# c5shen/WITCH

Measured on AMD Instinct MI355X. Metric: query-seqs aligned/sec (100k queries x 200-HMM eHMM), higher is better.
Workload: dtype f32; 1 GPU; dna_100k_x200; n_queries=100000, n_hmms=200, query_len=150, model_len_min=898, model_len_max=993, k=10, pairs_reported_rank0=20000000, pairs_multidomain_rank0=968, pairs_long_list_rank0=0, pairs_dense_redo_rank0=3, topk_crc32=3263627139

## Files before the change

### include/witch_hip.h

```cpp
#ifndef WITCH_HIP_H
#define WITCH_HIP_H

#include <stdint.h>

#ifdef __cplusplus
extern "C" {
#endif

#define WH_OK          0
#define WH_EINVAL     -1
#define WH_EIO        -2
#define WH_ENODEV     -3
#define WH_EHIP       -4
#define WH_ERANGE     -5
#define WH_ENOMEM     -6

#define WH_ALPH_DNA    0
#define WH_ALPH_RNA    1
#define WH_ALPH_AMINO  2

#define WH_FLAG_REPORTED  1
#define WH_FLAG_MULTI     2
#define WH_FLAG_OVERRIDE  4
#define WH_FLAG_TRUNC     8
// ... 141 lines not shown
int wh_last_score_counters(wh_ehmm *e, int64_t *out8);
int wh_last_region_overflow(wh_ehmm *e, int64_t *out4);
int wh_last_long_query_pairs(wh_ehmm *e, int64_t out[2]);
int wh_last_long_score_pairs(wh_ehmm *e, int64_t out[2]);
int wh_last_long_align_pairs(wh_ehmm *e, int64_t out[2]);

int wh_set_path_buffer(wh_ehmm *e, uint8_t *d_paths);
int wh_set_path_buffer16(wh_ehmm *e, uint16_t *d_paths);

int wh_last_queue_reruns(wh_ehmm *e);

int wh_consensus(wh_ehmm *e, const int64_t *offsets, int64_t nq, const int64_t *qpair_off,
                 const int32_t *pair_h, const double *pair_w, const int64_t *col_offsets, const int32_t *cols,
                 const int64_t *ret_off, const int32_t *retained, const int32_t *nongaps,
                 int32_t backbone_length, int32_t *out, int32_t *minmax);
int wh_consensus_dev(wh_ehmm *e, const int64_t *d_offsets, int64_t nq, int32_t max_len, const int64_t *d_qpair_off,
                     const int32_t *d_pair_h, const double *d_pair_w, const int64_t *d_col_offsets,
                     const int32_t *d_cols, const int64_t *d_ret_off, const int32_t *d_retained,
                     const int32_t *d_nongaps, int32_t backbone_length, int32_t max_pairs_per_query,
                     int32_t *d_out, int32_t *d_minmax, void *stream);

int wh_last_kernel_ms(wh_ehmm *e, int which, double *ms, int *launches);
int wh_last_score_launches(wh_ehmm *e, int32_t *cells_per_lane, int32_t *kind, double *ms, int cap);
int wh_set_timing(wh_ehmm *e, int enabled);
int wh_set_option(wh_ehmm *e, const char *name, const char *value);

int wh_merge(int device, const uint8_t *q_text, const int64_t *q_off, int64_t nq, const int32_t *codes, const int32_t *q_row,
             const uint8_t *backbone, int32_t nb, int32_t B, uint8_t **out_full, uint8_t **out_masked, int64_t *out_rows,
             int64_t *out_width);
int wh_merge_sharded(int device, const uint8_t *q_text, const int64_t *q_off, int64_t nq, const int32_t *codes, const int32_t *q_row,
                     const uint8_t *backbone, int32_t nb, int32_t B, int32_t *widths_local, const int32_t *widths_global,
                     uint8_t **out_full, uint8_t **out_masked, int64_t *out_rows, int64_t *out_width);

#define WH_MSA_TRIM   1
#define WH_MSA_NO_LDS 2
#define WH_MSA_CONS_HMMER 4
int wh_msa(wh_ehmm *e, const uint8_t *residues, const int64_t *offsets, const uint8_t *text, int64_t nq, int32_t h,
           int32_t flags, int64_t *out_W, uint8_t **out_rows, uint8_t **out_pp_rows, uint8_t **out_pp_cons, uint8_t **out_rf,
           int32_t **out_matmap, int64_t *out_pathless);
int wh_msa_dev(wh_ehmm *e, const int32_t *d_cols, const float *d_pp, const uint8_t *d_text, const int64_t *d_offsets,
               int64_t nq, int64_t total_residues, int32_t h, int32_t flags, int64_t *out_W, uint8_t **out_rows,
               uint8_t **out_pp_rows, uint8_t **out_pp_cons, uint8_t **out_rf, int32_t **out_matmap, int64_t *out_pathless,
               void *stream);

int wh_msa_mapali(wh_ehmm *e, const uint8_t *residues, const int64_t *offsets, const uint8_t *text, int64_t nq, int32_t h,
                  int32_t flags, const uint8_t *map_rows, int64_t n_map, int64_t alen, int64_t *out_W, uint8_t **out_rows,
// ... 90 lines not shown
```

### witch_amd/_lib.py

```python
from __future__ import annotations

import ctypes as C
import os
import subprocess

_HERE = os.path.dirname(os.path.abspath(__file__))
LIB_PATH = os.path.join(_HERE, "libwitch_hip.so")
CSRC = os.path.join(_HERE, "csrc")

WH_MAX_ENVELOPES = 16
FLAG_REPORTED, FLAG_MULTI, FLAG_OVERRIDE, FLAG_TRUNC, FLAG_EXACT = 1, 2, 4, 8, 16
FLAG_FILTERED = 32
BIAS_FILTER_ON = 2
STAGE_MSV, STAGE_BIAS, STAGE_VIT, STAGE_VIT_RAN, STAGE_FWD = 1, 2, 4, 8, 16
VIT_NOT_RUN, VIT_OVERFLOW, MSV_OVERFLOW = -32769, 32768, -1
ALPH_DNA, ALPH_RNA, ALPH_AMINO = 0, 1, 2
WH_OK, WH_EINVAL, WH_EIO, WH_ENODEV, WH_EHIP, WH_ERANGE, WH_ENOMEM = 0, -1, -2, -3, -4, -5, -6
WH_BUILD_STATS, WH_BUILD_CALIB_NO_LDS = 1, 4
WH_MSA_TRIM, WH_MSA_NO_LDS, WH_MSA_CONS_HMMER = 1, 2, 4
WH_LENMODEL_ENVELOPE, WH_LENMODEL_SEQUENCE = 0, 1
PATH_P2_WIN, PATH_P2_FULL, PATH_P4_W256, PATH_P4_W512, PATH_P4_WFAIL, PATH_P4_FULL, PATH_DENSE, PATH_MULTI = 1, 2, 4, 8, 16, 32, 64, 128


class WitchHipError(RuntimeError):
# ... 118 lines not shown
    "wh_seq_expect": (C.c_int, [_P, _P, _P, C.c_int64, _P, C.c_int64, _P]),
    "wh_seq_expect_dev": (C.c_int, [_P, _P, _P, C.c_int64, C.c_int64, C.c_int32, _P, C.c_int64, _P, _P]),
    "wh_seq_expect_host": (C.c_int, [C.POINTER(C.c_char_p), C.c_int, _P, _P, C.c_int64, _P, C.c_int64, _P]),
    "wh_seq_table": (C.c_int, [_P, _P, _P, C.c_int64, _P, _P, _P, _P, C.c_int64]),
    "wh_seq_table_dev": (C.c_int, [_P, _P, _P, C.c_int64, C.c_int64, C.c_int32, _P, _P, _P, _P, C.c_int64, _P]),
    "wh_seq_table_host": (C.c_int, [C.c_int, _P, _P, _P, C.c_int64, _P, _P, _P, _P, _P, C.c_int64]),
    "wh_last_seq_table_status": (C.c_int, [_P, _P]),
    "wh_ehmm_evparams": (C.c_int, [_P, _P, _P, _P]),
    "wh_hmm_evparams": (C.c_int, [C.c_char_p, C.POINTER(C.c_float), C.POINTER(C.c_float), C.POINTER(C.c_int32)]),
    "wh_consensus": (C.c_int, [_P, _P, C.c_int64, _P, _P, _P, _P, _P, _P, _P, _P, C.c_int32, _P, _P]),
    "wh_consensus_dev": (C.c_int, [_P, _P, C.c_int64, C.c_int32, _P, _P, _P, _P, _P, _P, _P, _P, C.c_int32, C.c_int32, _P, _P, _P]),
    "wh_last_align_status": (C.c_int, [_P, C.POINTER(C.c_int64), C.POINTER(C.c_int64), _P, C.c_int64]),
    "wh_last_align_paths": (C.c_int, [_P, _P]),
    "wh_last_score_paths": (C.c_int, [_P, _P]),
    "wh_last_score_counters": (C.c_int, [_P, _P]),
    "wh_set_path_buffer": (C.c_int, [_P, _P]),
    "wh_set_path_buffer16": (C.c_int, [_P, _P]),
    "wh_last_queue_reruns": (C.c_int, [_P]),
    "wh_last_region_overflow": (C.c_int, [_P, _P]),
    "wh_last_long_query_pairs": (C.c_int, [_P, _P]),
    "wh_last_long_score_pairs": (C.c_int, [_P, _P]),
    "wh_last_long_align_pairs": (C.c_int, [_P, _P]),
    "wh_last_score_launches": (C.c_int, [_P, _P, _P, _P, C.c_int]),
    "wh_last_kernel_ms": (C.c_int, [_P, C.c_int, C.POINTER(C.c_double), C.POINTER(C.c_int)]),
    "wh_set_timing": (C.c_int, [_P, C.c_int]),
    "wh_set_option": (C.c_int, [_P, C.c_char_p, C.c_char_p]),
}

_LIB = None


def build(force: bool = False, verbose: bool = False) -> str:
    cmd = ["make", "-C", CSRC, "-j4"] + (["-B"] if force else [])
    r = subprocess.run(cmd, stdout=subprocess.PIPE, stderr=subprocess.STDOUT, text=True)
    if verbose or r.returncode != 0:
        print(r.stdout)
    if r.returncode != 0:
        raise WitchHipError("building libwitch_hip.so failed:\n" + r.stdout[-4000:])
    return LIB_PATH


def lib():
    global _LIB
    if _LIB is None:
        if not os.path.exists(LIB_PATH):
            raise WitchHipError(
# ... 20 lines not shown
```

### witch_amd/csrc/wh_api.hip

```cpp
#include <atomic>
#include <chrono>
#include <memory>
#include <thread>

#include "wh_host.h"

static int g_device = -1;

extern "C" {

const char *wh_version(void) { return "witch_hip 0.1.0 (gfx950)"; }
const char *wh_last_error(void) { return wh::last_error(); }

int wh_init(int device) {
  int n = 0;
  if (hipGetDeviceCount(&n) != hipSuccess || n <= 0) {
    set_error("no HIP device visible");
    return WH_ENODEV;
  }
  if (device < 0 || device >= n) {
    set_error("device %d out of range (0..%d)", device, n - 1);
    return WH_EINVAL;
  }
  HIPCHK(hipSetDevice(device));
// ... 278 lines not shown
  out[0] = e->last_long_align[0]; out[1] = e->last_long_align[1];
  return WH_OK;
}

int wh_last_queue_reruns(wh_ehmm *e) {
  if (!e) { set_error("wh_last_queue_reruns: null handle"); return WH_EINVAL; }
  return e->last_queue_reruns;
}

int wh_last_score_launches(wh_ehmm *e, int32_t *cells_per_lane, int32_t *kind, double *ms, int cap) {
  if (!e || cap < 0) { set_error("wh_last_score_launches: bad argument"); return WH_EINVAL; }
  const int n = e->cls_n > 0 ? e->cls_n - 1 : 0;
  for (int t = 0; t < n && t < cap; t++) {
    HIPCHK(hipEventSynchronize(e->cls_ev[(size_t)t + 1]));
    float f = 0.f;
    HIPCHK(hipEventElapsedTime(&f, e->cls_ev[(size_t)t], e->cls_ev[(size_t)t + 1]));
    if (cells_per_lane) cells_per_lane[t] = e->cls_q[(size_t)t];
    if (kind) kind[t] = e->cls_kind[(size_t)t];
    if (ms) ms[t] = f;
  }
  return n;
}

int wh_last_kernel_ms(wh_ehmm *e, int which, double *ms, int *launches) {
  if (!e || which < 0 || which >= wh_ehmm::kTimers) return WH_EINVAL;
  KernelTimer &t = e->timers[which];
  if (t.pending) {
    HIPCHK(hipEventSynchronize(t.e1));
    float f = 0.f;
    HIPCHK(hipEventElapsedTime(&f, t.e0, t.e1));
    t.ms = f;
    t.pending = false;
  }
  if (ms) *ms = t.ms;
  if (launches) *launches = t.launches;
  return WH_OK;
}

int wh_merge(int device, const uint8_t *q_text, const int64_t *q_off, int64_t nq, const int32_t *codes, const int32_t *q_row,
             const uint8_t *backbone, int32_t nb, int32_t B, uint8_t **out_full, uint8_t **out_masked, int64_t *out_rows,
             int64_t *out_width) {
  return wh_merge_sharded(device, q_text, q_off, nq, codes, q_row, backbone, nb, B, nullptr, nullptr, out_full, out_masked, out_rows, out_width);
}

int wh_merge_sharded(int device, const uint8_t *q_text, const int64_t *q_off, int64_t nq, const int32_t *codes, const int32_t *q_row,
                     const uint8_t *backbone, int32_t nb, int32_t B, int32_t *widths_local, const int32_t *widths_global,
// ... 281 lines not shown
```

### witch_amd/csrc/wh_host.h

```cpp
#pragma once
#include <hip/hip_runtime.h>

#include <algorithm>
#include <cmath>
#include <cstdio>
#include <cstdlib>
#include <cstring>
#include <map>
#include <memory>
#include <vector>

#include "wh_devbuf.h"
#include "wh_knobs.h"
#include "wh_launch.h"
#include "wh_plan.h"

namespace wh {
const char *last_error();
}

using namespace wh;

struct KernelTimer {
  hipEvent_t e0 = nullptr, e1 = nullptr;
// ... 89 lines not shown
  uint16_t *path_buf16 = nullptr;
  static const int kStagingSlots = 11;
  DevBuf staging[kStagingSlots];
  DevBuf d_rkeys, d_rorder, d_rchunks, d_qorder, d_order, d_items, d_recs, d_spec, d_back, d_cwj, d_cwv, d_cwn, d_crow;
  uint32_t degen[32];
  struct FilterStateDelete { void operator()(FilterState *f) const; };
  std::unique_ptr<FilterState, FilterStateDelete> filter;
  struct SeqTabStateDelete { void operator()(SeqTabState *f) const; };
  std::unique_ptr<SeqTabState, SeqTabStateDelete> seqtab;
  struct DisplayStateDelete { void operator()(DisplayState *f) const; };
  std::unique_ptr<DisplayState, DisplayStateDelete> display;
  bool timing = false;
  static const int kTimers = 10;
  KernelTimer timers[kTimers];
  int max_M = 0;
  int max_Q = 4;
  int last_align_redo = 0;
  int last_align_unaligned = 0;
  int64_t last_align_paths[4] = {0, 0, 0, 0};
  std::vector<int64_t> last_unaligned_pairs;
  std::vector<hipEvent_t> cls_ev;
  std::vector<int> cls_q, cls_kind;
  int cls_n = 0;
  int *counter(int slot) const { return (int *)d_counter.p + slot; }
  ResolveFeedback *d_feedback() const { return (ResolveFeedback *)counter(kSlotResolveFeedback); }
};

static inline int max_query_len(const int64_t *offsets, int64_t nq) {
  int64_t m = 0;
  for (int64_t i = 0; i < nq; i++) m = std::max(m, offsets[i + 1] - offsets[i]);
  return (int)m;
}
static inline int check_residues(int Kp, const uint8_t *residues, int64_t total) {
  for (int64_t i = 0; i < total; i++)
    if (residues[i] >= Kp) { set_error("residue code %d at position %lld is not in the alphabet", residues[i], (long long)i); return WH_EINVAL; }
  return WH_OK;
}

struct Staging {
  wh_ehmm *e;
  int rc = WH_OK, next = 0, nback = 0;
  struct { void *host; const void *dev; size_t bytes; } back[wh_ehmm::kStagingSlots];
  explicit Staging(wh_ehmm *handle) : e(handle) {}
  template <class T> const T *in(const T *host, size_t bytes, size_t pad = 0) { return (const T *)take((void *)host, bytes, pad, true, false); }
  template <class T> T *out(T *host, size_t bytes, size_t pad = 0) { return (T *)take(host, bytes, pad, false, true); }
  template <class T> T *inout(T *host, size_t bytes, size_t pad = 0) { return (T *)take(host, bytes, pad, true, true); }
// ... 169 lines not shown
```

### witch_amd/csrc/wh_host_score.hip

```cpp
#include "wh_host.h"

static const int kStagedMaxBatches = 1 << 15;
static const int kStagedQB = 48;

static int resolve_main_cap(int max_M) {
  const size_t per_wave = (kLdsBudget - resolve_lds_header_bytes(0)) / (size_t)resolve_waves_per_cu();
  int lo = 1, hi = 1 << 20;
  while (lo < hi) {
    const int mid = lo + (hi - lo + 1) / 2;
    if (resolve_lds_bytes(mid, max_M) <= per_wave) lo = mid; else hi = mid - 1;
  }
  return lo;
}

static ScoreCall score_call(wh_ehmm *e, const uint8_t *d_residues, const int64_t *d_offsets, int64_t nq, int64_t total_residues, int32_t max_len,
                            int32_t *d_decibits, uint8_t *d_flags, float *d_fwd_bits, wh_pair_detail *d_detail, void *stream) {
  ScoreCall c = {e, (hipStream_t)stream, d_residues, d_offsets, nq, total_residues, max_len, d_decibits, d_flags, d_fwd_bits, d_detail};
  c.Lc = std::max(max_len, 1);
  c.H = (int)e->hmms.size();
  c.npairs_all = nq * (int64_t)c.H;
  const bool fits = resolve_lds_bytes(c.Lc, e->max_M) <= kLdsBudget;
  c.Lmain = fits || e->knobs.no_long_query ? c.Lc : resolve_main_cap(e->max_M);
  c.resolve = !e->knobs.no_resolve && (fits || !e->knobs.no_long_query) && c.npairs_all < 0x7FFFFFFF;
  c.mixed = nq > 0 && total_residues > 0 && (double)max_len > 1.25 * (double)total_residues / (double)nq;
  c.wide_dense = getenv("WH_WIDE_DENSE"); c.wide_no_em_lds = getenv("WH_WIDE_NO_EM_LDS"); c.p2win_force = getenv("WH_P2WIN_FORCE");
  c.res_null2_gather = getenv("WH_RES_NULL2_GATHER"); c.res_no_lds_tables = getenv("WH_RES_NO_LDS_TABLES");
  if (const char *wv = getenv("WH_RES_WAVES")) c.res_waves = std::max(1, atoi(wv));
  c.Ls = main_length_cap(e, c.Lc, false, c.resolve, c.p2win_force);
  return c;
}

struct StagedWaves { int wl, one, both, p2, p4; };
enum class ScoreFamily { PhaseCall, PhaseCallB, TwoQuery, FourEnvelope, PassSync, Staged };
static const char *const kFamilyName[] = {"phase-call", "phase-call(B)", "two-queries-per-wave", "phase-call", "pass-synchronous", "staged"};

struct ScoreClassPlan {
  int Q, list_off, n_list;
  ScoreFamily family;
  LdsPlan b;
  int Klds;
  bool specg;
  int p2win;
  bool use_qorder;
  int QB, n_qblocks, n_items;
  size_t scratch_stride, spec_stride;
  int blocks;
  StagedWaves st;
};

static int cap_waves(const Knobs &kn, int w) { return cap_waves(kn.max_waves, w); }
static size_t score_table_bytes(const wh_ehmm *e, int Q) { return score_table_bytes(e->K, Q); }

static const int G_all = 1, G_most = 4, G_few = 8, G_rare = 32;
static int staged_cand_cap(int G, int per_pair) { return std::min(G * kStagedQB * per_pair, 2048); }
static size_t staged_lds(int Q, int wl, int arrays, int waves, int cand) {
  return lds_bytes(kLdsHeader + (size_t)cand * sizeof(int), (size_t)arrays * Q * kWave * sizeof(float), waves, wl);
}
// ... 17 lines not shown
  const size_t table = score_table_bytes(e, Q);
  ScoreClassPlan p = {};
  p.Q = Q; p.list_off = list_off; p.n_list = n_list;
  ScoreLds l;
  if (!plan_score_lds(plan_knobs(e, c.p2win_force), e->K, Q, Lc, true, &l)) { set_error("query length %d with model class Q=%d does not fit in LDS", c.max_len, Q); return WH_ERANGE; }
  p.b = l.b; p.Klds = l.Klds;
  LdsPlan &b = p.b;
  const bool big = l.big, specg = l.specg, pairk = l.pairk, p2win = l.p2win, p2inpl = l.p2inpl;
  bool quadk = false;
  if ((kn.kernel == 10 || kn.kernel == 11) && !e->st_off && !big && !pairk && !specg && !kn.dbg && (Q == 8 || Q == 12 || Q == 16 || Q == 20 || Q == 24) &&
      plan_staged(e, Q, Lc, &p.st)) {
    p.family = ScoreFamily::Staged;
    b.SP = row_stride(Lc); b.wave_lds = p.st.wl;
    p.QB = kStagedQB; p.n_qblocks = (int)((nq + p.QB - 1) / p.QB); p.n_items = n_list * p.n_qblocks;
    p.scratch_stride = (size_t)(Lc + 1) * 2 * Q * kWave;
    *out = p;
    return WH_OK;
  }
  if (kn.kernel == 12 && !big && !pairk && !specg && Q == 16) {
    const int wlq = kScoreSpecArrays * row_stride(Lc) + 128 + kRegsInts + 4 * 16 + 4 * 16 + 4 * residue_words(Lc);
    const int wq = fit_waves(kLdsHeader, table, cap_waves(kn, 12), wlq);
    if (wq >= 8) { quadk = true; b = {wq, row_stride(Lc), wlq, lds_bytes(kLdsHeader, table, wq, wlq)}; }
  }
  p.family = big ? ScoreFamily::PassSync : pairk ? ScoreFamily::TwoQuery : quadk ? ScoreFamily::FourEnvelope : kn.kernel == 8 ? ScoreFamily::PhaseCallB : ScoreFamily::PhaseCall;
  p.p2win = (specg || big || pairk || quadk) ? 0 : p2win ? 1 : p2inpl ? 2 : 0;
  p.use_qorder = big || c.mixed;
  const int waves = b.waves;
  p.QB = big ? waves * 2 : pairk ? waves * 4 : waves * (kn.item_g > 0 ? kn.item_g : 32);
  const int per_turn = pairk ? 2 : 1;
  const int max_blocks = big ? e->cu_count : e->cu_count * std::max(1, 8 / waves);
  if ((int64_t)n_list * ((nq + p.QB - 1) / p.QB) < 4 * (int64_t)max_blocks) {
    p.QB = waves * per_turn;
    if (!big && !pairk) for (int g_ = 16; g_ > 1; g_ /= 2)
      if ((int64_t)n_list * ((nq + waves * g_ - 1) / (waves * g_)) >= 4 * (int64_t)max_blocks) { p.QB = waves * g_; break; }
  }
  if (quadk) p.QB = std::max(p.QB, waves * 8);
  p.n_qblocks = (int)((nq + p.QB - 1) / p.QB);
  p.n_items = n_list * p.n_qblocks;
  p.scratch_stride = (size_t)(quadk ? 5 : per_turn) * (size_t)(Lc + 1) * 2 * Q * kWave;
  p.spec_stride = specg ? (size_t)8 * b.SP : quadk ? (size_t)(5 * kScoreSpecArrays + 1) * b.SP : 0;
  p.specg = specg || quadk;
  p.blocks = clamp_blocks(std::min(p.n_items, max_blocks), (size_t)waves * (p.scratch_stride + p.spec_stride) * sizeof(float), e->d_scratch, e->max_M, Lc, "scoring");
  if (p.blocks < 0) return WH_ENOMEM;
  *out = p;
  return WH_OK;
}

static ScoreArgs class_args(const ScoreCall &c, const ScoreClassPlan &p, int launches) {
  const wh_ehmm *e = c.e;
  const Knobs &kn = e->knobs;
  ScoreArgs a;
  fill_common(a, c);
  a.tables = (const float *)e->d_tables.p;
  a.hmm_list = (const int32_t *)e->d_lists.p + p.list_off; a.n_list = p.n_list;
  a.counter = e->counter(kSlotLaunch0 + launches);
  a.dbg = kn.dbg;
  a.no_window = kn.no_window ? 1 : 0;
  a.keep_scale = kn.keep_scale;
  a.spill_band = kn.kernel != 9 ? kn.spill_band : 0;
  a.Klds = p.Klds; a.SP = p.b.SP; a.wave_lds = p.b.wave_lds; a.spec_arrays = kScoreSpecArrays;
  if (p.family == ScoreFamily::PhaseCall || p.family == ScoreFamily::FourEnvelope) a.spec_arrays |= kScoreSpecLayout << 8;
  a.paths = reinterpret_cast<unsigned long long *>(e->counter(kSlotScorePath));
  a.p2win = p.p2win;
  a.qorder = p.use_qorder ? c.d_qorder : nullptr;
  a.QB = p.QB; a.n_qblocks = p.n_qblocks; a.n_items = p.n_items;
  a.scratch_stride = p.scratch_stride; a.spec_stride = p.spec_stride;
  a.scratch = (float *)e->d_scratch.p;
  if (p.specg) a.spec_scratch = (float *)e->d_spec.p;
  return a;
}

static int print_class_stats(const ScoreCall &c, int Q, const unsigned long long *stats) {
  unsigned long long st[40];
  if (int rc = stats_read(c, stats, st)) return rc;
  const double tot = (double)(st[4] + st[5] + st[6] + st[7] + st[8] + st[9] + st[10] + st[11]);
  fprintf(stderr, "[wh] Q=%d wave cycles: P1 %.1f%%  P2 %.1f%%  regions %.1f%%  P3 %.1f%%  P4 %.1f%%  null2 %.1f%%  swaps+barriers %.1f%%  other %.1f%%  (total %.3g ticks)\n", Q, 100.0 * st[4] / tot,
          100.0 * st[5] / tot, 100.0 * st[6] / tot, 100.0 * st[7] / tot, 100.0 * st[8] / tot, 100.0 * st[9] / tot, 100.0 * st[10] / tot, 100.0 * st[11] / tot, tot);
  if (st[38]) fprintf(stderr, "[wh] Q=%d wave lifetimes %.3g cycles: %.1f%% in the phases above, %.1f%% fetching an item (two barriers)\n", Q, (double)st[38], 100.0 * tot / (double)st[38], 100.0 * (double)st[39] / (double)st[38]);
  if (st[37]) fprintf(stderr, "[wh] Q=%d four-envelope sweeps: %llu envelopes, %.0f wave cycles per envelope (slot 'null2' above)\n", Q, st[37], (double)st[9] / (double)st[37]);
  fprintf(stderr, "[wh] Q=%d envelope Backward sweeps: %llu on a 256-node window, %llu on a 512-node window, %llu windows failed the mass certificate, %llu full width; union of the stored lane blocks: span %.1f blocks (with margin), %.1f blocks set, of %llu envelopes\n", Q, st[0], st[1], st[2], st[3], (double)st[12] / (double)std::max(1ull, st[14]), (double)st[15] / (double)std::max(1ull, st[14]), st[14]);
  fprintf(stderr, "[wh] Q=%d multihit Backward on a window: %llu scans, of them in doubt at a threshold %llu, at the multidomain bound %llu; window loss out of range %llu; mean eps %.3g\n", Q,
          st[35], st[32], st[33], st[36], st[35] ? 1e-9 * (double)st[34] / (double)st[35] : 0.0);
  fprintf(stderr, "[wh] Q=%d |Ld - mass| / Ld  (<3e-7, <1e-6, <3e-6, <1e-5, <2e-5, more): window sweeps %llu %llu %llu %llu %llu %llu; full-width sweeps %llu %llu %llu %llu %llu %llu\n", Q,
          st[16], st[17], st[18], st[19], st[20], st[21], st[22], st[23], st[24], st[25], st[26], st[27]);
  return WH_OK;
}

static int launch_score_class(const ScoreCall &c, const ScoreClassPlan &p, int *launches) {
  wh_ehmm *e = c.e;
  hipStream_t s = c.s;
  const int Q = p.Q, waves = p.b.waves, threads = waves * kWave;
  const bool big = p.family == ScoreFamily::PassSync;
  ScoreArgs a = class_args(c, p, *launches);
  if (a.p2win == 2) {
    a.p2_backup_stride = (size_t)kScoreSpecArrays * a.SP;
    if (e->d_p2bak.ensure((size_t)p.blocks * waves * a.p2_backup_stride * sizeof(float))) return WH_ENOMEM;
    a.p2_backup = (float *)e->d_p2bak.p;
  }
  if (int rc = stats_begin(c, 320, 13, &a.stats)) return rc;
  if (e->knobs.trace) fprintf(stderr, "[wh] score Q=%d kernel=%s specg=%d waves=%d blocks=%d lds=%zu SP=%d wave_lds=%d items=%d Lcap=%d\n", Q,
                              kFamilyName[(int)p.family], (int)p.specg, waves, p.blocks, p.b.lds, a.SP, a.wave_lds, a.n_items, a.Lcap);
  HIPCHK(hipMemsetAsync(a.counter, 0, sizeof(int), s));
  if (class_mark(e, s, Q, big ? 1 : 0)) return WH_EHIP;
  hipError_t err = big ? launch_score_big(Q, a, p.blocks, threads, p.b.lds, s)
                   : p.family == ScoreFamily::TwoQuery ? launch_score9(Q, a, p.blocks, threads, p.b.lds, s)
                   : p.family == ScoreFamily::FourEnvelope ? launch_score7q(Q, a, p.blocks, threads, p.b.lds, s)
                   : p.family == ScoreFamily::PhaseCallB ? launch_score7b(Q, a, p.blocks, threads, p.b.lds, s)
                                                         : launch_score7(Q, a, p.blocks, threads, p.b.lds, s);
  if (err != hipSuccess) { set_error("score kernel launch (Q=%d) failed: %s", Q, hipGetErrorString(err)); return WH_EHIP; }
  (*launches)++;
  return a.stats ? print_class_stats(c, Q, a.stats) : WH_OK;
}

static int print_staged_stats(const ScoreCall &c, int Q, const unsigned long long *stats) {
  unsigned long long st[64];
  if (int rc = stats_read(c, stats, st)) return rc;
  static const char *kind[9] = {"p1", "p2win 256", "p2win 512", "p2full", "p3", "p4win 256", "p4win 512", "p4full", "dense"};
  for (int k = 0; k < 9; k++)
    fprintf(stderr, "[wh] staged Q=%d %-10s sweeps %9llu  shader cycles per sweep %10.0f  real time per sweep %8.1f us  (clock %.2f GHz)  wave lifetimes %.3g cycles, in sweeps %.1f%%\n", Q, kind[k], st[4 * k + 3],
            st[4 * k + 3] ? (double)st[4 * k] / (double)st[4 * k + 3] : 0.0, st[4 * k + 3] ? 0.01 * (double)st[4 * k + 1] / (double)st[4 * k + 3] : 0.0,
            st[4 * k + 1] ? 0.1 * (double)st[4 * k] / (double)st[4 * k + 1] : 0.0, (double)st[4 * k + 2], st[4 * k + 2] ? 100.0 * (double)st[4 * k] / (double)st[4 * k + 2] : 0.0);
  return WH_OK;
}

static int launch_staged_class(const ScoreCall &c, const ScoreClassPlan &p, int *launches) {
  wh_ehmm *e = c.e;
  hipStream_t s = c.s;
  const Knobs &kn = e->knobs;
  const bool split = kn.kernel == 11;
  const int Q = p.Q, Lc = c.Ls, K = e->K, w_one = p.st.one, w_both = p.st.both, w_p2 = p.st.p2, w_p4 = p.st.p4;
// ... 238 lines not shown
    most_units = std::max(most_units, e->st_cnt_host[(size_t)32 * b + ST_N_UNITS]);
  }
  if (!*over && most_units > 0 && e->st_last_NB > 0) e->st_upp = std::max(1.05, 1.25 * (double)most_units / (double)e->st_last_NB);
  if (!*over) return WH_OK;
  if (e->knobs.trace) fprintf(stderr, "[wh] staged launches: a batch ran out of envelope units, the scoring pass is repeated with the fused kernel\n");
  e->st_upp = std::min<double>(WH_MAX_ENVELOPES, e->st_upp * 2.0);
  e->st_off = true;
  return WH_OK;
}

static void prefetch_align_workspace(const ScoreCall &c) {
  wh_ehmm *e = c.e;
  const size_t need = (size_t)8 * (size_t)e->cu_count * (size_t)(c.Ls + 1) * 5 * (size_t)e->by_q.rbegin()->first * kWave * sizeof(float);
  size_t free_b = 0, total_b = 0;
  if (need > e->d_ascratch.cap && hipMemGetInfo(&free_b, &total_b) == hipSuccess && need < free_b / 10) (void)e->d_ascratch.ensure(need);
}

static int score_dev_pass(ScoreCall &c, bool *overflow) {
  wh_ehmm *e = c.e;
  hipStream_t s = c.s;
  HIPCHK(hipSetDevice(e->device));
  if (timer_begin(e, 0, s)) return WH_EHIP;
  e->cls_n = 0;
  e->last_staged_batches = 0;
  int launches = 0;
  bool wide_done = false;
  if (c.nq > 0) {
    if ((int)e->by_q.size() > kMaxLaunches) { set_error("too many model size classes (%zu)", e->by_q.size()); return WH_ERANGE; }
    if (int rc = size_resolver_queue(c)) return rc;
    HIPCHK(hipMemsetAsync(e->counter(kSlotScorePath), 0, kScorePathInts * sizeof(int), s));
    static_assert(2 * kPathRecSlot + 2 == kScorePathInts, "the record's address takes the last of the eight path counters");
    if (e->path_buf16) HIPCHK(hipMemcpyAsync(e->counter(kSlotScorePath) + 2 * kPathRecSlot, &e->path_buf16, sizeof e->path_buf16, hipMemcpyHostToDevice, s));
    if (int rc = order_queries(c)) return rc;
    if (int rc = score_size_classes(c, &launches)) return rc;
    if (!e->wide_by_w.empty()) if (int rc = score_wide_classes(c, &launches, &wide_done)) return rc;
    if (!e->generic_front.empty() || (!wide_done && !e->wide_by_w.empty() && !e->force_wide))
      if (int rc = score_front_end(c, wide_done, &launches)) return rc;
  }
  if (class_mark(e, s, 0, -1)) return WH_EHIP;
  if (timer_end(e, 0, s, launches)) return WH_EHIP;
  if (e->last_staged_batches > 0) {
    bool over = false;
    if (int rc = read_staged_counters(c, &over)) return rc;
    if (over) {
      *overflow = true;
      if (timer_begin(e, 4, s) || timer_end(e, 4, s, 0)) return WH_EHIP;
// ... 55 lines not shown
```

### witch_amd/csrc/wh_launch.h

```cpp
#pragma once
#include <hip/hip_runtime.h>

#include <cstddef>

#include "wh_common.h"

namespace wh {

struct ResolveRec {
  int64_t q;
  int32_t h;
  float fwdsc;
  float fwd_bits;
  int32_t nreg;
  int32_t nenv;
  int32_t flags;
  int32_t multi_mask;
  int32_t ri[WH_MAX_ENVELOPES], rj[WH_MAX_ENVELOPES];
  float envsc[WH_MAX_ENVELOPES], domcorr[WH_MAX_ENVELOPES];
};

struct ScoreArgs {
  const DevHMM *hmms;
  const float *tables;
// ... 74 lines not shown
  StPair *pairs;
  float *p1spec; size_t p1stride;
  StUnit *units;
  float *p3spec; size_t p3stride;
  float *slabs; size_t slab_stride;
  int *cnt;
  uint8_t *pair_paths;
  uint16_t *pair_paths16;
};
constexpr int kStWantedWindow = 1 << 16;
hipError_t launch_staged_p1(int Q, const StagedArgs &a, int blocks, int threads, size_t lds, hipStream_t s);
hipError_t launch_staged_p2win(int Q, int QB, const StagedArgs &a, int blocks, int threads, size_t lds, hipStream_t s);
hipError_t launch_staged_p2full(int Q, const StagedArgs &a, int blocks, int threads, size_t lds, hipStream_t s);
hipError_t launch_staged_p3(int Q, const StagedArgs &a, int blocks, int threads, size_t lds, hipStream_t s);
hipError_t launch_staged_p4win(int Q, int QB, const StagedArgs &a, int blocks, int threads, size_t lds, hipStream_t s);
hipError_t launch_staged_p4full(int Q, const StagedArgs &a, int blocks, int threads, size_t lds, hipStream_t s);
hipError_t launch_staged_dense(int Q, const StagedArgs &a, int blocks, int threads, size_t lds, hipStream_t s);
hipError_t launch_staged_env(int Q, const StagedArgs &a, int blocks, int threads, size_t lds, hipStream_t s);
hipError_t launch_staged_assemble(const StagedArgs &a, hipStream_t s);

hipError_t launch_score_big(int Q, const ScoreArgs &a, int blocks, int threads, size_t lds, hipStream_t s);
hipError_t launch_score7(int Q, const ScoreArgs &a, int blocks, int threads, size_t lds, hipStream_t s);
hipError_t launch_score7b(int Q, const ScoreArgs &a, int blocks, int threads, size_t lds, hipStream_t s);
hipError_t launch_score7q(int Q, const ScoreArgs &a, int blocks, int threads, size_t lds, hipStream_t s);
hipError_t launch_score9(int Q, const ScoreArgs &a, int blocks, int threads, size_t lds, hipStream_t s);
int score9_block_floats(int SP, int Lcap);

struct ResolveFeedback {
  int wrong_model;
  int long_list_pairs;
  int big_pairs, big_doms, big_segs, big_clus;
  int long_pairs, longest_query;
  int big_cap;
  int long_cap;
  int32_t *big_list, *long_list;
};
constexpr size_t kFeedbackUploadFrom = offsetof(ResolveFeedback, big_pairs);

struct ResolveArgs {
  const DevHMM *hmms;
  const double *gtab;
  const float *ftab;
  const uint8_t *residues;
  const int64_t *offsets;
  const ResolveRec *recs;
  const int32_t *order;
// ... 414 lines not shown
```

### witch_amd/csrc/wh_plan.h

```cpp
#pragma once
#include <algorithm>
#include <cstddef>
#include <vector>

#include "wh_common.h"

namespace wh {

size_t wide_lds_bytes(int Lcap, size_t em_floats);
size_t generic_lds_bytes(int Lcap);
int score9_block_floats(int SP, int Lcap);

constexpr size_t kLdsBudget = 160 * 1024 - 512;
constexpr size_t kLdsHeader = 16;
constexpr int kScoreSpecArrays = 6;
#ifndef WH_K7_LAYOUT
#define WH_K7_LAYOUT 1
#endif
constexpr int kScoreSpecLayout = WH_K7_LAYOUT;
constexpr int kAlignSpecRows = 14;
constexpr int kMaxPlanLength = 1 << 24;

inline int row_stride(int Lc) { return (Lc + 1 + 3) / 4 * 4; }
inline int residue_words(int Lc) { return (Lc + 3) / 4 + 4; }
inline size_t lds_bytes(size_t header, size_t table, int w, int wave_words) { return header + table + (size_t)w * (size_t)wave_words * sizeof(float); }
inline int fit_waves(size_t header, size_t table, int w, int wave_words, int per_cu = 1) {
  while (w >= 1 && per_cu * lds_bytes(header, table, w, wave_words) > kLdsBudget) w--;
  return w;
}
inline bool plan_long_model(int Q, int K, int wave_words, int *Klds, size_t *lds) {
  *Klds = K;
  size_t table = (size_t)(K + 8) * Q * kWave * sizeof(float);
  if (lds_bytes(kLdsHeader, table, 4, wave_words) > kLdsBudget) { *Klds = 0; table = (size_t)8 * Q * kWave * sizeof(float); }
  *lds = lds_bytes(kLdsHeader, table, 4, wave_words);
  return *lds <= kLdsBudget;
}

struct PlanKnobs { int kernel = 7, max_waves = 0; bool force_specg = false, no_window = false, no_p2win = false, p2win_force = false; };
struct LdsPlan { int waves, SP, wave_lds; size_t lds; };
inline int cap_waves(int max_waves, int w) { return max_waves > 0 ? std::max(1, std::min(w, max_waves)) : w; }
inline size_t score_table_bytes(int K, int Q) { return (size_t)(K + 2 * FW_NARR) * Q * kWave * sizeof(float); }

inline bool plan_block1(int max_waves, int K, int Q, int Lcap, int extra_arrays, LdsPlan *b) {
  const int sp = row_stride(Lcap);
  const int wl = (kScoreSpecArrays + extra_arrays) * sp + 32 + kRegsInts + residue_words(Lcap);
  const int w = fit_waves(kLdsHeader, score_table_bytes(K, Q), cap_waves(max_waves, 12), wl);
  if (w < 1) return false;
  *b = {w, sp, wl, lds_bytes(kLdsHeader, score_table_bytes(K, Q), w, wl)};
  return true;
}

struct ScoreLds { LdsPlan b; bool big, specg, pairk, p2win, p2inpl; int Klds; };
inline bool plan_score_lds(const PlanKnobs &kn, int K, int Q, int Lc, bool with9, ScoreLds *out) {
  const size_t table = score_table_bytes(K, Q);
  ScoreLds r = {};
  LdsPlan &b = r.b;
  r.big = Q > kMaxQFast;
  if (with9 && !r.big && kn.kernel == 9 && !kn.force_specg && (Q == 8 || Q == 12 || Q == 16)) {
    const int wl9 = 2 * score9_block_floats(row_stride(Lc), Lc), w9 = cap_waves(kn.max_waves, 8);
    if (lds_bytes(kLdsHeader, table, w9, wl9) <= kLdsBudget) { r.pairk = true; b = {w9, row_stride(Lc), wl9, lds_bytes(kLdsHeader, table, w9, wl9)}; }
  }
  if (!r.big && !r.pairk) {
    bool ok = plan_block1(kn.max_waves, K, Q, Lc, 0, &b);
    if (ok && b.waves >= 4 && !kn.force_specg && !kn.no_window && !kn.no_p2win && Q >= 8) {
      LdsPlan b2 = {};
      if (plan_block1(kn.max_waves, K, Q, Lc, 3, &b2) && (b2.waves >= b.waves || (kn.p2win_force && b2.waves >= 8))) { r.p2win = true; b = b2; }
      else if (Q >= 20 && kn.kernel != 9) r.p2inpl = true;
    }
    if (!ok || b.waves < 4 || kn.force_specg) {
      r.specg = true;
      b.SP = row_stride(Lc);
      b.wave_lds = 32 + kRegsInts + residue_words(Lc);
      b.waves = fit_waves(kLdsHeader, table, cap_waves(kn.max_waves, Q <= 16 ? 12 : 8), b.wave_lds);
      ok = b.waves >= 1;
      b.lds = lds_bytes(kLdsHeader, table, b.waves, b.wave_lds);
      if (Q >= 20 && (!ok || b.waves < 4)) r.big = true;
      if (Q == 16 && !ok) r.big = true;
    }
    if (!r.big && !ok) return false;
  }
  if (r.big) {
    b.waves = 4; b.SP = row_stride(Lc); b.wave_lds = 32 + kRegsInts + residue_words(Lc);
    if (!plan_long_model(Q, K, b.wave_lds, &r.Klds, &b.lds)) return false;
    r.specg = true;
  }
  *out = r;
  return true;
}

struct AlignLds { int waves, SP, wave_lds, Klds; size_t lds; bool spec_in_hbm, swap; };
// ... 72 lines not shown
```

### witch_amd/csrc/wh_score7.hip

```cpp
#include <hip/hip_runtime.h>

#include "wh_device.h"
#include "wh_launch.h"

#ifndef WH_K7NS
#define WH_K7NS k7
#define WH_K7LAUNCH launch_score7
#endif

namespace wh {
namespace WH_K7NS {


constexpr float kKeepScale7 = 5.9604645e-08f;
constexpr float kMassTol7 = 2e-5f;
constexpr float kWinTol7 = 3e-6f;
__device__ __forceinline__ float spill_tol(bool banded) { return banded ? kWinTol7 : kMassTol7; }
#ifndef WH_K7_MAXQP
#define WH_K7_MAXQP 0
#endif
constexpr int kMaxQP = WH_K7_MAXQP;
#ifdef WH_SLIM_SPEC
constexpr bool kSlim = true;
constexpr int kSpML = SP_B, kSpMH = SP_E, kSpArr = 6;
// ... 13 lines not shown
#ifndef WH_UNI
#define WH_UNI WH_K7_NEW_DEFAULT
#endif
#ifndef WH_ROW_PAIRS
#define WH_ROW_PAIRS (WH_K7_NEW_DEFAULT ? 3 : 0)
#endif
#ifndef WH_SPLIT_SLACK
#define WH_SPLIT_SLACK 1
#endif
#ifndef WH_ROW_WAITS
#define WH_ROW_WAITS (WH_K7_NEW_DEFAULT ? 3 : 0)
#endif
#ifndef WH_ROW_AHEAD
#define WH_ROW_AHEAD (WH_K7_NEW_DEFAULT ? 7 : 0)
#endif
constexpr int kLayout = WH_SPEC_ROWS ? SPEC_ROWS : SPEC_SOA;
constexpr bool kUni = WH_UNI != 0;
constexpr bool kRowPairs = ((WH_ROW_PAIRS) & 1) != 0, kUniArgs = ((WH_ROW_PAIRS) & 2) != 0, kSplitSlack = WH_SPLIT_SLACK != 0;
constexpr bool kDrain = ((WH_ROW_WAITS) & 1) != 0, kLateRequest = ((WH_ROW_WAITS) & 2) != 0;
constexpr bool kAheadCode = ((WH_ROW_AHEAD) & 1) != 0, kAheadPiece = ((WH_ROW_AHEAD) & 3) == 3, kAheadWrites = ((WH_ROW_AHEAD) & 4) != 0;
static_assert(kLayout == SPEC_SOA || kSlim, "a row record has six words (WH_SLIM_SPEC)");
template <bool SG> using SpecOf = SpecAt<SG ? (int)SPEC_SOA : kLayout>;
constexpr int kSpecTag = kSpArr | (kLayout << 8);

__device__ __noinline__ static double dlog(double x) { return log(x); }
__device__ __noinline__ static double dexp(double x) { return exp(x); }
__device__ __forceinline__ float flogsum0_v7(float b) {
  const float mx = b > 0.f ? b : 0.f, mn = b > 0.f ? 0.f : b;
  if (mn == -INFINITY || (mx - mn) >= 15.7f) return mx;
  const int idx = (int)((mx - mn) * 1000.0f);
  return mx + (float)dlog(1.0 + dexp((double)-idx / 1000.0));
}

typedef __attribute__((address_space(3))) float lds_f;
typedef __attribute__((address_space(3))) uint8_t lds_u8;
typedef __attribute__((address_space(3))) int lds_i;
typedef __attribute__((address_space(1))) float glb_f;

struct WaveCtx {
  lds_f *emL;
  const glb_f *emG;
  lds_f *fwL, *bwL;
  lds_f *spec;
  glb_f *specg;
  lds_f *n2tab;
  glb_f *Fs;
// ... 1235 lines not shown
      wh_pair_detail *dp = (a.detail && lane == 0) ? a.detail + out : nullptr;
      if (dp) {
        dp->fwd_bits = -INFINITY; dp->seq_score = 0.f; dp->pre_score = 0.f; dp->seqbias_nats = 0.f;
        dp->nregions = 0; dp->nenv = 0;
      }
      if (L > 0 && L <= a.Lcap) {
        for (int t = lane; t < L; t += kWave) {
          int r = a.residues[off + t];
          seq[t] = (uint8_t)(r < a.Kp ? r : a.Kp - 1);
        }
        __builtin_amdgcn_wave_barrier();
        long long t_last = a.stats ? __builtin_readcyclecounter() : 0;
        const LenCfg cm = len_config(L, true);
        const FwdOut f1 = uniform_fwd(sweep_forward<Q, false, TH, SG>(c, (lds_u8 *)seq, L, cm, 0.f));
        const double fwd_nats = (double)f1.ef * LOG2 + dlog((double)(f1.xC * cm.move));
        const float fwdsc = uniform_f((float)fwd_nats);
        const float p1 = (float)L / (float)(L + 1);
        const float nullsc = uniform_f((float)((double)(float)L * dlog((double)p1) + dlog(1.0 - (double)p1)));
        fwd_bits_out = uniform_f((float)((fwd_nats - (double)nullsc) / LOG2));
        if (dp) dp->fwd_bits = fwd_bits_out;
        if (f1.xC > 0.f && isfinite(fwdsc)) {
          WH_TICK7(4);
          RegOut ro;
          if constexpr (!SG && Q >= 20) {
            if (a.p2win == 2) ro = score_regions<Q, TH, false, true>(a, c, seq, regs, L, lane, cm, f1, fs, t_last, (glb_f *)(a.p2_backup + ((size_t)blockIdx.x * nwaves + wave) * a.p2_backup_stride));
            else ro = score_regions<Q, TH, SG, false>(a, c, seq, regs, L, lane, cm, f1, fs, t_last);
          } else ro = score_regions<Q, TH, SG, false>(a, c, seq, regs, L, lane, cm, f1, fs, t_last);
          const int nenv = ro.nenv, nreg = ro.nreg, multi_mask = ro.flags >> 8;
          flags |= ro.flags & 0xFF;
          if (dp) { dp->nregions = nreg; dp->nenv = nenv; }
          if (nenv > 0) {
            WH_TICK7(6);
            score_envelopes<Q, TH, SG>(a, c, seq, regs, L, lane, h, qi, nenv, nreg, multi_mask, fwdsc, nullsc, fwd_bits_out, dp, flags, decibits, ec, t_last, p1_mask(c));
          }
        }
      }
      if (lane == 0) {
        a.decibits[out] = decibits;
        a.flags[out] = (uint8_t)flags;
        if (a.fwd_bits) a.fwd_bits[out] = fwd_bits_out;
      }
      const unsigned band_ev = take_band_events(ec);
      if (uint16_t *rec = path_record(a)) {
        if (lane == 0) rec[out] = (uint16_t)path_bits(regs, ec, fs, isfinite(fwd_bits_out), flags, (flags & WH_FLAG_MULTI) && a.rrecs != nullptr, band_ev);
      }
    }
  }
// ... 286 lines not shown

template <int Q, int TH>
static hipError_t launch7(const ScoreArgs &a, int blocks, int threads, size_t lds, hipStream_t s) {
  if (a.spec_scratch) return launch7sg<Q, TH, true>(a, blocks, threads, lds, s);
  return launch7sg<Q, TH, false>(a, blocks, threads, lds, s);
}

template <int TH>
static hipError_t launch7_q(int Q, const ScoreArgs &a, int blocks, int threads, size_t lds, hipStream_t s) {
  switch (Q) {
    case 4:  return launch7<4, TH>(a, blocks, threads, lds, s);
    case 8:  return launch7<8, TH>(a, blocks, threads, lds, s);
    case 12: return launch7<12, TH>(a, blocks, threads, lds, s);
    case 16: return launch7<16, TH>(a, blocks, threads, lds, s);
    case 20: return launch7<20, TH>(a, blocks, threads, lds, s);
    case 24: return launch7<24, TH>(a, blocks, threads, lds, s);
    default: return hipErrorInvalidValue;
  }
}

#endif
}

#if !defined(WH_SWEEPS_ONLY) && !defined(WH_K7B)
hipError_t launch_score7q(int Q, const ScoreArgs &a, int blocks, int threads, size_t lds, hipStream_t s) {
  using namespace WH_K7NS;
  if (a.spec_arrays != kSpecTag || !a.spec_scratch || threads > 768) return hipErrorInvalidValue;
  if (Q == 16) return launch7q<16, 768>(a, blocks, threads, lds, s);
  return hipErrorInvalidValue;
}
#endif
#ifndef WH_SWEEPS_ONLY
hipError_t WH_K7LAUNCH(int Q, const ScoreArgs &a, int blocks, int threads, size_t lds, hipStream_t s) {
  using namespace WH_K7NS;
  if (!a.spec_scratch && a.spec_arrays != kSpecTag) return hipErrorInvalidValue;
  if (threads <= 512) return launch7_q<512>(Q, a, blocks, threads, lds, s);
  if (threads <= 768) return launch7_q<768>(Q, a, blocks, threads, lds, s);
  return hipErrorInvalidValue;
}
#endif

}
```

### witch_amd/ehmm.py

```python
from __future__ import annotations

import ctypes as C

import numpy as np

from . import _lib
from ._lib import BIAS_FILTER_ON, DOMAIN_FIELDS, FilterOpts, PairDetail, WitchHipError, check, lib


def pack_queries(seqs):
    offs = np.zeros(len(seqs) + 1, dtype=np.int64)
    if len(seqs):
        offs[1:] = np.cumsum([len(s) for s in seqs])
        res = np.concatenate([np.asarray(s, dtype=np.uint8) for s in seqs])
    else:
        res = np.zeros(0, dtype=np.uint8)
    return np.ascontiguousarray(res), offs


def alignment_checksum(molecule, rows):
    rows = [r.encode() if isinstance(r, str) else bytes(r) for r in rows]
    if not rows or len(set(len(r) for r in rows)) != 1:
        raise ValueError("alignment_checksum: the rows must be of one length")
    out = C.c_uint32(0)
# ... 127 lines not shown
        if model not in self._LENGTH_MODELS:
            raise ValueError("domain length model %r: one of %s" % (model, ", ".join(map(repr, self._LENGTH_MODELS))))
        check(lib().wh_set_domain_length_model(self._h, self._LENGTH_MODELS.index(model)), "wh_set_domain_length_model")

    @property
    def domain_length_model(self) -> str:
        v = lib().wh_get_domain_length_model(self._h)
        if v < 0:
            check(v, "wh_get_domain_length_model")
        return self._LENGTH_MODELS[v]

    def last_kernel_ms(self, which: int):
        ms, n = C.c_double(0), C.c_int(0)
        check(lib().wh_last_kernel_ms(self._h, which, C.byref(ms), C.byref(n)), "wh_last_kernel_ms")
        return ms.value, n.value

    def last_score_launches(self):
        q = np.zeros(64, dtype=np.int32)
        kind = np.zeros(64, dtype=np.int32)
        ms = np.zeros(64, dtype=np.float64)
        n = lib().wh_last_score_launches(self._h, q.ctypes.data, kind.ctypes.data, ms.ctypes.data, 64)
        check(min(n, 0), "wh_last_score_launches")
        return [(int(q[t]), int(kind[t]), float(ms[t])) for t in range(min(n, 64))]

    def last_score_paths(self):
        p6 = np.zeros(6, dtype=np.int64)
        check(lib().wh_last_score_paths(self._h, p6.ctypes.data), "wh_last_score_paths")
        return {"window256": int(p6[0]), "window512": int(p6[1]), "window_rejected": int(p6[2]), "full_width": int(p6[3]),
                "p2_window": int(p6[4]), "p2_window_in_doubt": int(p6[5])}

    def last_score_spill_bytes(self) -> int:
        c8 = np.zeros(8, dtype=np.int64)
        check(lib().wh_last_score_counters(self._h, c8.ctypes.data), "wh_last_score_counters")
        return int(c8[6])

    def last_long_list_pairs(self) -> int:
        c8 = np.zeros(8, dtype=np.int64)
        check(lib().wh_last_score_counters(self._h, c8.ctypes.data), "wh_last_score_counters")
        return int(c8[7])

    def last_region_overflow(self):
        o4 = np.zeros(4, dtype=np.int64)
        check(lib().wh_last_region_overflow(self._h, o4.ctypes.data), "wh_last_region_overflow")
        return {"pairs": int(o4[0]), "max_domains": int(o4[1]), "max_segments": int(o4[2]), "max_clusters": int(o4[3])}

    def last_long_queries(self):
# ... 617 lines not shown
```

Baseline: 26150 queries/s.

## Add 16-wave phase-call score kernel variant for mid-size query classes

Adds a PhaseCallW score family that plans a 1024-thread block (16 waves) for Q=8/12/16 classes when the LDS plan fits. By default only the Q=16 class qualifies. That class drops the p2 window and uses the in-place region path with a global backup, which a new build flag enables for Q>=8. The aim is to fit more waves per block and shared score-table LDS so more queries run concurrently. The cost is extra global backup traffic and a heavier register/LDS footprint per block. A small API is also added to report the per-launch score shapes.

```diff
diff --git a/include/witch_hip.h b/include/witch_hip.h
--- a/include/witch_hip.h
+++ b/include/witch_hip.h
@@ -187,6 +187,7 @@
 
 int wh_last_kernel_ms(wh_ehmm *e, int which, double *ms, int *launches);
 int wh_last_score_launches(wh_ehmm *e, int32_t *cells_per_lane, int32_t *kind, double *ms, int cap);
+int wh_last_score_shapes(wh_ehmm *e, int32_t *cells_per_lane, int32_t *waves, int32_t *p2win, int cap);
 int wh_set_timing(wh_ehmm *e, int enabled);
 int wh_set_option(wh_ehmm *e, const char *name, const char *value);
 
diff --git a/witch_amd/_lib.py b/witch_amd/_lib.py
--- a/witch_amd/_lib.py
+++ b/witch_amd/_lib.py
@@ -164,6 +164,7 @@
     "wh_last_long_score_pairs": (C.c_int, [_P, _P]),
     "wh_last_long_align_pairs": (C.c_int, [_P, _P]),
     "wh_last_score_launches": (C.c_int, [_P, _P, _P, _P, C.c_int]),
+    "wh_last_score_shapes": (C.c_int, [_P, _P, _P, _P, C.c_int]),
     "wh_last_kernel_ms": (C.c_int, [_P, C.c_int, C.POINTER(C.c_double), C.POINTER(C.c_int)]),
     "wh_set_timing": (C.c_int, [_P, C.c_int]),
     "wh_set_option": (C.c_int, [_P, C.c_char_p, C.c_char_p]),
diff --git a/witch_amd/csrc/wh_api.hip b/witch_amd/csrc/wh_api.hip
--- a/witch_amd/csrc/wh_api.hip
+++ b/witch_amd/csrc/wh_api.hip
@@ -324,6 +324,17 @@
   return n;
 }
 
+int wh_last_score_shapes(wh_ehmm *e, int32_t *cells_per_lane, int32_t *waves, int32_t *p2win, int cap) {
+  if (!e || cap < 0) { set_error("wh_last_score_shapes: bad argument"); return WH_EINVAL; }
+  const int n = (int)e->last_shapes.size();
+  for (int t = 0; t < n && t < cap; t++) {
+    if (cells_per_lane) cells_per_lane[t] = e->last_shapes[(size_t)t].q;
+    if (waves) waves[t] = e->last_shapes[(size_t)t].waves;
+    if (p2win) p2win[t] = e->last_shapes[(size_t)t].p2win;
+  }
+  return n;
+}
+
 int wh_last_kernel_ms(wh_ehmm *e, int which, double *ms, int *launches) {
   if (!e || which < 0 || which >= wh_ehmm::kTimers) return WH_EINVAL;
   KernelTimer &t = e->timers[which];
diff --git a/witch_amd/csrc/wh_host.h b/witch_amd/csrc/wh_host.h
--- a/witch_amd/csrc/wh_host.h
+++ b/witch_amd/csrc/wh_host.h
@@ -135,6 +135,8 @@
   std::vector<hipEvent_t> cls_ev;
   std::vector<int> cls_q, cls_kind;
   int cls_n = 0;
+  struct ScoreShape { int q, waves, p2win; };
+  std::vector<ScoreShape> last_shapes;
   int *counter(int slot) const { return (int *)d_counter.p + slot; }
   ResolveFeedback *d_feedback() const { return (ResolveFeedback *)counter(kSlotResolveFeedback); }
 };
diff --git a/witch_amd/csrc/wh_host_score.hip b/witch_amd/csrc/wh_host_score.hip
--- a/witch_amd/csrc/wh_host_score.hip
+++ b/witch_amd/csrc/wh_host_score.hip
@@ -31,8 +31,8 @@
 }
 
 struct StagedWaves { int wl, one, both, p2, p4; };
-enum class ScoreFamily { PhaseCall, PhaseCallB, TwoQuery, FourEnvelope, PassSync, Staged };
-static const char *const kFamilyName[] = {"phase-call", "phase-call(B)", "two-queries-per-wave", "phase-call", "pass-synchronous", "staged"};
+enum class ScoreFamily { PhaseCall, PhaseCallB, TwoQuery, FourEnvelope, PassSync, Staged, PhaseCallW };
+static const char *const kFamilyName[] = {"phase-call", "phase-call(B)", "two-queries-per-wave", "phase-call", "pass-synchronous", "staged", "phase-call(16 waves)"};
 
 struct ScoreClassPlan {
   int Q, list_off, n_list;
@@ -96,7 +96,8 @@
     const int wq = fit_waves(kLdsHeader, table, cap_waves(kn, 12), wlq);
     if (wq >= 8) { quadk = true; b = {wq, row_stride(Lc), wlq, lds_bytes(kLdsHeader, table, wq, wlq)}; }
   }
-  p.family = big ? ScoreFamily::PassSync : pairk ? ScoreFamily::TwoQuery : quadk ? ScoreFamily::FourEnvelope : kn.kernel == 8 ? ScoreFamily::PhaseCallB : ScoreFamily::PhaseCall;
+  p.family = big ? ScoreFamily::PassSync : pairk ? ScoreFamily::TwoQuery : quadk ? ScoreFamily::FourEnvelope : kn.kernel == 8 ? ScoreFamily::PhaseCallB
+             : l.four ? ScoreFamily::PhaseCallW : ScoreFamily::PhaseCall;
   p.p2win = (specg || big || pairk || quadk) ? 0 : p2win ? 1 : p2inpl ? 2 : 0;
   p.use_qorder = big || c.mixed;
   const int waves = b.waves;
@@ -133,7 +134,7 @@
   a.keep_scale = kn.keep_scale;
   a.spill_band = kn.kernel != 9 ? kn.spill_band : 0;
   a.Klds = p.Klds; a.SP = p.b.SP; a.wave_lds = p.b.wave_lds; a.spec_arrays = kScoreSpecArrays;
-  if (p.family == ScoreFamily::PhaseCall || p.family == ScoreFamily::FourEnvelope) a.spec_arrays |= kScoreSpecLayout << 8;
+  if (p.family == ScoreFamily::PhaseCall || p.family == ScoreFamily::PhaseCallW || p.family == ScoreFamily::FourEnvelope) a.spec_arrays |= kScoreSpecLayout << 8;
   a.paths = reinterpret_cast<unsigned long long *>(e->counter(kSlotScorePath));
   a.p2win = p.p2win;
   a.qorder = p.use_qorder ? c.d_qorder : nullptr;
@@ -175,11 +176,13 @@
   if (e->knobs.trace) fprintf(stderr, "[wh] score Q=%d kernel=%s specg=%d waves=%d blocks=%d lds=%zu SP=%d wave_lds=%d items=%d Lcap=%d\n", Q,
                               kFamilyName[(int)p.family], (int)p.specg, waves, p.blocks, p.b.lds, a.SP, a.wave_lds, a.n_items, a.Lcap);
   HIPCHK(hipMemsetAsync(a.counter, 0, sizeof(int), s));
+  e->last_shapes.push_back({Q, waves, a.p2win});
   if (class_mark(e, s, Q, big ? 1 : 0)) return WH_EHIP;
   hipError_t err = big ? launch_score_big(Q, a, p.blocks, threads, p.b.lds, s)
                    : p.family == ScoreFamily::TwoQuery ? launch_score9(Q, a, p.blocks, threads, p.b.lds, s)
                    : p.family == ScoreFamily::FourEnvelope ? launch_score7q(Q, a, p.blocks, threads, p.b.lds, s)
                    : p.family == ScoreFamily::PhaseCallB ? launch_score7b(Q, a, p.blocks, threads, p.b.lds, s)
+                   : p.family == ScoreFamily::PhaseCallW ? launch_score7w(Q, a, p.blocks, threads, p.b.lds, s)
                                                          : launch_score7(Q, a, p.blocks, threads, p.b.lds, s);
   if (err != hipSuccess) { set_error("score kernel launch (Q=%d) failed: %s", Q, hipGetErrorString(err)); return WH_EHIP; }
   (*launches)++;
@@ -464,6 +467,7 @@
   HIPCHK(hipSetDevice(e->device));
   if (timer_begin(e, 0, s)) return WH_EHIP;
   e->cls_n = 0;
+  e->last_shapes.clear();
   e->last_staged_batches = 0;
   int launches = 0;
   bool wide_done = false;
diff --git a/witch_amd/csrc/wh_launch.h b/witch_amd/csrc/wh_launch.h
--- a/witch_amd/csrc/wh_launch.h
+++ b/witch_amd/csrc/wh_launch.h
@@ -120,6 +120,7 @@
 hipError_t launch_score_big(int Q, const ScoreArgs &a, int blocks, int threads, size_t lds, hipStream_t s);
 hipError_t launch_score7(int Q, const ScoreArgs &a, int blocks, int threads, size_t lds, hipStream_t s);
 hipError_t launch_score7b(int Q, const ScoreArgs &a, int blocks, int threads, size_t lds, hipStream_t s);
+hipError_t launch_score7w(int Q, const ScoreArgs &a, int blocks, int threads, size_t lds, hipStream_t s);
 hipError_t launch_score7q(int Q, const ScoreArgs &a, int blocks, int threads, size_t lds, hipStream_t s);
 hipError_t launch_score9(int Q, const ScoreArgs &a, int blocks, int threads, size_t lds, hipStream_t s);
 int score9_block_floats(int SP, int Lcap);
diff --git a/witch_amd/csrc/wh_plan.h b/witch_amd/csrc/wh_plan.h
--- a/witch_amd/csrc/wh_plan.h
+++ b/witch_amd/csrc/wh_plan.h
@@ -41,16 +41,22 @@
 inline int cap_waves(int max_waves, int w) { return max_waves > 0 ? std::max(1, std::min(w, max_waves)) : w; }
 inline size_t score_table_bytes(int K, int Q) { return (size_t)(K + 2 * FW_NARR) * Q * kWave * sizeof(float); }
 
-inline bool plan_block1(int max_waves, int K, int Q, int Lcap, int extra_arrays, LdsPlan *b) {
+inline bool plan_block1(int max_waves, int K, int Q, int Lcap, int extra_arrays, LdsPlan *b, int top = 12) {
   const int sp = row_stride(Lcap);
   const int wl = (kScoreSpecArrays + extra_arrays) * sp + 32 + kRegsInts + residue_words(Lcap);
-  const int w = fit_waves(kLdsHeader, score_table_bytes(K, Q), cap_waves(max_waves, 12), wl);
+  const int w = fit_waves(kLdsHeader, score_table_bytes(K, Q), cap_waves(max_waves, top), wl);
   if (w < 1) return false;
   *b = {w, sp, wl, lds_bytes(kLdsHeader, score_table_bytes(K, Q), w, wl)};
   return true;
 }
 
-struct ScoreLds { LdsPlan b; bool big, specg, pairk, p2win, p2inpl; int Klds; };
+constexpr int kFourWaveClasses = 1 << 4;
+inline bool four_wave_class(int max_waves, int Q) {
+  if (Q != 8 && Q != 12 && Q != 16) return false;
+  return max_waves == 16 || (max_waves == 0 && ((kFourWaveClasses >> (Q / 4)) & 1));
+}
+
+struct ScoreLds { LdsPlan b; bool big, specg, pairk, p2win, p2inpl; int Klds; bool four; };
 inline bool plan_score_lds(const PlanKnobs &kn, int K, int Q, int Lc, bool with9, ScoreLds *out) {
   const size_t table = score_table_bytes(K, Q);
   ScoreLds r = {};
@@ -66,6 +72,10 @@
       LdsPlan b2 = {};
       if (plan_block1(kn.max_waves, K, Q, Lc, 3, &b2) && (b2.waves >= b.waves || (kn.p2win_force && b2.waves >= 8))) { r.p2win = true; b = b2; }
       else if (Q >= 20 && kn.kernel != 9) r.p2inpl = true;
+    }
+    if (ok && b.waves >= 4 && !kn.force_specg && !kn.no_window && !kn.no_p2win && kn.kernel == 7 && four_wave_class(kn.max_waves, Q)) {
+      LdsPlan b4 = {};
+      if (plan_block1(kn.max_waves, K, Q, Lc, 0, &b4, 16) && b4.waves == 16) { r.four = true; r.p2win = false; r.p2inpl = true; b = b4; }
     }
     if (!ok || b.waves < 4 || kn.force_specg) {
       r.specg = true;
diff --git a/witch_amd/csrc/wh_score7.hip b/witch_amd/csrc/wh_score7.hip
--- a/witch_amd/csrc/wh_score7.hip
+++ b/witch_amd/csrc/wh_score7.hip
@@ -59,6 +59,11 @@
 static_assert(kLayout == SPEC_SOA || kSlim, "a row record has six words (WH_SLIM_SPEC)");
 template <bool SG> using SpecOf = SpecAt<SG ? (int)SPEC_SOA : kLayout>;
 constexpr int kSpecTag = kSpArr | (kLayout << 8);
+#ifdef WH_K7W
+constexpr int kInPlaceMinQ = 8;
+#else
+constexpr int kInPlaceMinQ = 20;
+#endif
 
 __device__ __noinline__ static double dlog(double x) { return log(x); }
 __device__ __noinline__ static double dexp(double x) { return exp(x); }
@@ -1340,7 +1345,7 @@
         if (f1.xC > 0.f && isfinite(fwdsc)) {
           WH_TICK7(4);
           RegOut ro;
-          if constexpr (!SG && Q >= 20) {
+          if constexpr (!SG && Q >= kInPlaceMinQ) {
             if (a.p2win == 2) ro = score_regions<Q, TH, false, true>(a, c, seq, regs, L, lane, cm, f1, fs, t_last, (glb_f *)(a.p2_backup + ((size_t)blockIdx.x * nwaves + wave) * a.p2_backup_stride));
             else ro = score_regions<Q, TH, SG, false>(a, c, seq, regs, L, lane, cm, f1, fs, t_last);
           } else ro = score_regions<Q, TH, SG, false>(a, c, seq, regs, L, lane, cm, f1, fs, t_last);
@@ -1673,7 +1678,7 @@
 #endif
 }
 
-#if !defined(WH_SWEEPS_ONLY) && !defined(WH_K7B)
+#if !defined(WH_SWEEPS_ONLY) && !defined(WH_K7B) && !defined(WH_K7W)
 hipError_t launch_score7q(int Q, const ScoreArgs &a, int blocks, int threads, size_t lds, hipStream_t s) {
   using namespace WH_K7NS;
   if (a.spec_arrays != kSpecTag || !a.spec_scratch || threads > 768) return hipErrorInvalidValue;
@@ -1681,7 +1686,18 @@
   return hipErrorInvalidValue;
 }
 #endif
-#ifndef WH_SWEEPS_ONLY
+#ifdef WH_K7W
+hipError_t WH_K7LAUNCH(int Q, const ScoreArgs &a, int blocks, int threads, size_t lds, hipStream_t s) {
+  using namespace WH_K7NS;
+  if (a.spec_scratch || a.spec_arrays != kSpecTag || threads != 1024) return hipErrorInvalidValue;
+  switch (Q) {
+    case 8:  return launch7sg<8, 1024, false>(a, blocks, threads, lds, s);
+    case 12: return launch7sg<12, 1024, false>(a, blocks, threads, lds, s);
+    case 16: return launch7sg<16, 1024, false>(a, blocks, threads, lds, s);
+    default: return hipErrorInvalidValue;
+  }
+}
+#elif !defined(WH_SWEEPS_ONLY)
 hipError_t WH_K7LAUNCH(int Q, const ScoreArgs &a, int blocks, int threads, size_t lds, hipStream_t s) {
   using namespace WH_K7NS;
   if (!a.spec_scratch && a.spec_arrays != kSpecTag) return hipErrorInvalidValue;
diff --git a/witch_amd/ehmm.py b/witch_amd/ehmm.py
--- a/witch_amd/ehmm.py
+++ b/witch_amd/ehmm.py
@@ -173,6 +173,12 @@
         n = lib().wh_last_score_launches(self._h, q.ctypes.data, kind.ctypes.data, ms.ctypes.data, 64)
         check(min(n, 0), "wh_last_score_launches")
         return [(int(q[t]), int(kind[t]), float(ms[t])) for t in range(min(n, 64))]
+
+    def last_score_shapes(self):
+        q, waves, p2win = (np.zeros(64, dtype=np.int32) for _ in range(3))
+        n = lib().wh_last_score_shapes(self._h, q.ctypes.data, waves.ctypes.data, p2win.ctypes.data, 64)
+        check(min(n, 0), "wh_last_score_shapes")
+        return [(int(q[t]), int(waves[t]), int(p2win[t])) for t in range(min(n, 64))]
 
     def last_score_paths(self):
         p6 = np.zeros(6, dtype=np.int64)
```

Result: faster. 27010 queries/s, median of 6 (+3.3%).
